# WhatAShot/Electrocardio-Panorama

Hardware: AMD Instinct MI355X
Metric: ECG-samples/sec (train step) (higher is better)
Workload: dtype f32 (conv products: fp32 operands split into fp16 hi+lo = 22-23 bits, block-scaled, 3 fp16 matrix products each, fp32 accumulate; fp32-class, not IEEE fp32)

## Files before the change

electrocardio_panorama_amd/csrc/conv_h2w.hip:

```cpp
#include <hip/hip_runtime.h>
#include <stdint.h>
#include <stdlib.h>

#include <type_traits>

#include "nefnet_hip.h"
#include "nef_common.h"


typedef float f32x16 __attribute__((ext_vector_type(16)));
typedef float f32x2 __attribute__((ext_vector_type(2)));
typedef _Float16 h16x8 __attribute__((ext_vector_type(8)));
typedef _Float16 h16x2 __attribute__((ext_vector_type(2)));
typedef unsigned u32x4 __attribute__((ext_vector_type(4)));
typedef unsigned u32x2 __attribute__((ext_vector_type(2)));

namespace {

constexpr int TT = 64;
constexpr int GP = TT * 2 + 8;
constexpr int XW = TT + 8;
constexpr int XP = XW * 2 + 8;
constexpr int X_PLANE = 64 * XP;
constexpr int gy_plane(int MCO) { return 64 * MCO * GP; }
constexpr int buf_bytes(int MCO) { return 2 * gy_plane(MCO) + 2 * X_PLANE; }

struct H2WArgs {
    const float* x;
    const float* gy;
    const float* in_scale;
    const float* pro_a;
    const float* pro_b;
    float* ws;
    const float* x_amax;
    const float* gy_amax;
    float* x_amax_next;
    float* gy_amax_next;
    int* clamped;
    int64_t x_bs, x_gs, gy_bs, gy_gs, sc_bs, sc_gs;
    int64_t x_end, gy_end;
    int B, T, G, Cig, Cog, pro_Bp, S, tps, n_tiles, m_tiles, c_tiles, teams;
    float x_scale, gy_scale;
    int xclamp;
};


__device__ __forceinline__ void split_pair_s(float x0, float x1, float s, unsigned& h, unsigned& l) {
    asm("v_fma_mixlo_f16 %0, %1, %2, 0 op_sel:[0,0,0] op_sel_hi:[0,0,0]" : "=v"(h) : "v"(x0), "v"(s));
    asm("v_fma_mixhi_f16 %0, %1, %2, 0 op_sel:[0,0,0] op_sel_hi:[0,0,0]" : "+v"(h) : "v"(x1), "v"(s));
    asm("v_fma_mixlo_f16 %0, %1, %2, -%3 op_sel:[0,0,0] op_sel_hi:[0,0,1]" : "=v"(l) : "v"(x0), "v"(s), "v"(h));
    asm("v_fma_mixhi_f16 %0, %1, %2, -%3 op_sel:[0,0,1] op_sel_hi:[0,0,1]" : "+v"(l) : "v"(x1), "v"(s), "v"(h));
}
__device__ __forceinline__ void split_one_s(float x0, float s, unsigned& h, unsigned& l) {
    asm("v_fma_mixlo_f16 %0, %1, %2, 0 op_sel:[0,0,0] op_sel_hi:[0,0,0]" : "=v"(h) : "v"(x0), "v"(s));
    asm("v_fma_mixlo_f16 %0, %1, %2, -%3 op_sel:[0,0,0] op_sel_hi:[0,0,1]" : "=v"(l) : "v"(x0), "v"(s), "v"(h));
}

__device__ __forceinline__ float scale_for(float m) {
    int e;
    (void)frexpf(m, &e);
    return ldexpf(1.f, 9 - e);
}

__device__ __forceinline__ float scale_from(const float* amax, float fallback) {
    float s = fallback != 0.f ? fallback : 1.f;
    if (amax) {
        const float m = amax[0];
        if (m > 0.f && m < 3e38f) {
            int e;
            (void)frexpf(m, &e);
            s = ldexpf(1.f, 9 - e);
        }
    }
    return s;
}

template <int K, int K0, int K1, int MCO, int KA>
__device__ __forceinline__ void h2w_chunk(const unsigned char* ga, const unsigned char* xa, int c, f32x16 (&acc)[MCO][KA]) {
    constexpr int PAD = (K - 1) / 2;
    constexpr int GY_PLANE = gy_plane(MCO);
    h16x8 fah[MCO], fal[MCO];
#pragma unroll
    for (int i = 0; i < MCO; ++i) {
        unsigned ah[4], al[4];
#pragma unroll
        for (int j = 0; j < 2; ++j) {
            const u32x2 vh = *reinterpret_cast<const u32x2*>(ga + i * 32 * GP + c * 32 + 8 * j);
            const u32x2 vl = *reinterpret_cast<const u32x2*>(ga + i * 32 * GP + GY_PLANE + c * 32 + 8 * j);
            ah[2 * j] = vh[0], ah[2 * j + 1] = vh[1];
            al[2 * j] = vl[0], al[2 * j + 1] = vl[1];
        }
        fah[i] = __builtin_bit_cast(h16x8, u32x4{ah[0], ah[1], ah[2], ah[3]});
        fal[i] = __builtin_bit_cast(h16x8, u32x4{al[0], al[1], al[2], al[3]});
    }
    unsigned wh[8], wl[8];
#pragma unroll
    for (int j = 0; j < 4; ++j) {
        const u32x2 vh = *reinterpret_cast<const u32x2*>(xa + c * 32 + 8 * j);
        const u32x2 vl = *reinterpret_cast<const u32x2*>(xa + X_PLANE + c * 32 + 8 * j);
        wh[2 * j] = vh[0], wh[2 * j + 1] = vh[1];
        wl[2 * j] = vl[0], wl[2 * j + 1] = vl[1];
    }
    __builtin_amdgcn_s_setprio(1);
#pragma unroll
    for (int k = K0; k < K1; ++k) {
        const int e0 = 4 + k - PAD;
        unsigned bh[4], bl[4];
#pragma unroll
        for (int j = 0; j < 4; ++j) {
            if ((e0 & 1) == 0) {
                bh[j] = wh[e0 / 2 + j];
                bl[j] = wl[e0 / 2 + j];
            } else {
                bh[j] = __builtin_amdgcn_alignbit(wh[(e0 + 1) / 2 + j], wh[(e0 - 1) / 2 + j], 16);
                bl[j] = __builtin_amdgcn_alignbit(wl[(e0 + 1) / 2 + j], wl[(e0 - 1) / 2 + j], 16);
            }
        }
        const h16x8 fbh = __builtin_bit_cast(h16x8, u32x4{bh[0], bh[1], bh[2], bh[3]});
        const h16x8 fbl = __builtin_bit_cast(h16x8, u32x4{bl[0], bl[1], bl[2], bl[3]});
#pragma unroll
        for (int i = 0; i < MCO; ++i) acc[i][k - K0] = __builtin_amdgcn_mfma_f32_32x32x16_f16(fah[i], fbh, acc[i][k - K0], 0, 0, 0);
#pragma unroll
        for (int i = 0; i < MCO; ++i) acc[i][k - K0] = __builtin_amdgcn_mfma_f32_32x32x16_f16(fah[i], fbl, acc[i][k - K0], 0, 0, 0);
#pragma unroll
        for (int i = 0; i < MCO; ++i) acc[i][k - K0] = __builtin_amdgcn_mfma_f32_32x32x16_f16(fal[i], fbh, acc[i][k - K0], 0, 0, 0);
    }
}

template <int K, int PRO, int MCO, int SPLIT>
__global__ __launch_bounds__(SPLIT ? 512 : 256, SPLIT ? 1 : 2) void conv_h2w_kernel(H2WArgs a) {
    constexpr bool UP = (PRO & 2) != 0, AFF = (PRO & 1) != 0;
    constexpr int NT = SPLIT ? 512 : 256;
    constexpr int ROWS_G = 64 * MCO;
    constexpr int GY_PLANE = gy_plane(MCO), BUF = buf_bytes(MCO);
    constexpr int KA = SPLIT == 1 ? (K + 1) / 2 : K;
    constexpr int NGQ = ROWS_G * (TT / 2) / NT;
    constexpr int NXQ = (64 * (XW / 2) + NT - 1) / NT;
    static_assert(SPLIT == 0 || MCO == 2, "the 512-thread forms are the 128-channel tile");
    extern __shared__ __attribute__((aligned(16))) unsigned char smem_w[];

    const int members = a.m_tiles * a.c_tiles;
    const int xcd = blockIdx.x & 7, q_ = blockIdx.x >> 3;
    const int member = q_ % members;
    const int team = (q_ / members) * 8 + xcd;
    if (team >= a.teams) return;
    const int g = team / a.S, sp = team % a.S;
    const int mt = member / a.c_tiles, ct = member % a.c_tiles;
    const int T = a.T, Tin = UP ? (T >> 1) : T;
    const int lane = threadIdx.x & 63, wave = threadIdx.x >> 6;
    const int lo = lane & 31, hi = lane >> 5;
    const int wave_u = __builtin_amdgcn_readfirstlane(wave);
    const int wt = wave_u >> 2;
    const int wm = (wave_u >> 1) & 1, wn = wave_u & 1;

    const int64_t per = ((int64_t)a.n_tiles + a.S - 1) / a.S;
    const int n_lo = (int)(per * sp);
    int n_hi = (int)(per * (sp + 1));
    if (n_hi > a.n_tiles) n_hi = a.n_tiles;

    float* const Wl = reinterpret_cast<float*>(smem_w);
    float rx_ = 0.f, rg_ = 0.f;
    auto share_pass = [&](const float sx, const float sg, const bool last) __attribute__((always_inline)) -> bool {
    float amax_x = 0.f, amax_g = 0.f;

    f32x16 acc[MCO][KA];
#pragma unroll
    for (int i = 0; i < MCO; ++i)
#pragma unroll
        for (int k = 0; k < KA; ++k)
#pragma unroll
            for (int r = 0; r < 16; ++r) acc[i][k][r] = 0.f;

    f32x2 gq[NGQ];
    f32x2 xq[NXQ][UP ? 2 : 1];
#define NEF_W_ISSUE(N)                                                                                               \
    {                                                                                                               \
        const int b_ = (N) / a.tps, t0_ = ((N) % a.tps) * TT;                                                       \
        const bool on_ = (N) < n_hi;                                                                                \
        const __amdgpu_buffer_rsrc_t grs = nef_rsrc_n(a.gy + (int64_t)b_ * a.gy_bs + (int64_t)g * a.gy_gs + (int64_t)(mt * ROWS_G) * T, \
                                                      on_ ? 0x7FFFFFFCu : 0u);                                      \
        _Pragma("unroll") for (int q = 0; q < NGQ; ++q) {                                                           \
            const int p = (int)threadIdx.x + NT * q;                                                                \
            const int row = p >> 5, t = t0_ + 2 * (p & 31);                                                         \
            gq[q] = nef_buf_f32x2(grs, t < T ? (unsigned)((row * T + t) * 4) : NEF_OOB, 0);                         \
        }                                                                                                           \
        const __amdgpu_buffer_rsrc_t xrs = nef_rsrc_n(a.x + (int64_t)b_ * a.x_bs + (int64_t)g * a.x_gs + (int64_t)(ct * 64) * Tin, \
                                                      on_ ? 0x7FFFFFFCu : 0u);                                      \
        _Pragma("unroll") for (int q = 0; q < NXQ; ++q) {                                                           \
            const int p = (int)threadIdx.x + NT * q;                                                                \
            const int row = p / (XW / 2), t = t0_ - 4 + 2 * (p % (XW / 2));                                         \
            const bool ok = p < 64 * (XW / 2) && t >= 0 && t < T;                                                   \
            if constexpr (UP) {                                                                                     \
                 \
                const int h_ = t >> 1;                                                                              \
                const int im = h_ > 0 ? h_ - 1 : 0, ip = h_ + 1 < Tin ? h_ + 1 : Tin - 1;                           \
                const float v0 = nef_buf_f32(xrs, ok ? (unsigned)((row * Tin + im) * 4) : NEF_OOB, 0);              \
                const float v1 = nef_buf_f32(xrs, ok ? (unsigned)((row * Tin + h_) * 4) : NEF_OOB, 0);              \
                const float v2 = nef_buf_f32(xrs, ok ? (unsigned)((row * Tin + ip) * 4) : NEF_OOB, 0);              \
                xq[q][0] = f32x2{v0, v1};                                                                           \
                xq[q][UP ? 1 : 0] = f32x2{v1, v2};                                                                  \
            } else {                                                                                                \
                xq[q][0] = nef_buf_f32x2(xrs, ok ? (unsigned)((row * T + t) * 4) : NEF_OOB, 0);                     \
            }                                                                                                       \
        }                                                                                                           \
    }
#define NEF_W_STORE(N, BUFP)                                                                                         \
    {                                                                                                               \
        const int b_ = (N) / a.tps, t0_ = ((N) % a.tps) * TT;                                                       \
        _Pragma("unroll") for (int q = 0; q < NGQ; ++q) {                                                           \
            const int p = (int)threadIdx.x + NT * q;                                                                \
            const int row = p >> 5, c2 = p & 31;                                                                    \
            amax_g = fmaxf(amax_g, fmaxf(fabsf(gq[q][0]), fabsf(gq[q][1])));                                        \
            unsigned h_, l_;                                                                                        \
            split_pair_s(gq[q][0], gq[q][1], sg, h_, l_);                                                           \
            unsigned char* p_ = (BUFP) + row * GP + c2 * 4;                                                         \
            *reinterpret_cast<unsigned*>(p_) = h_;                                                                  \
            *reinterpret_cast<unsigned*>(p_ + GY_PLANE) = l_;                                                       \
        }                                                                                                           \
        _Pragma("unroll") for (int q = 0; q < NXQ; ++q) {                                                           \
            const int p = (int)threadIdx.x + NT * q;                                                                \
            const int row = p / (XW / 2), c2 = p % (XW / 2), t = t0_ - 4 + 2 * c2;                                  \
            if (p < 64 * (XW / 2)) {                                                                                \
                const int ch = g * a.Cig + ct * 64 + row;                                                           \
                float v0, v1;                                                                                       \
                if constexpr (UP) {                                                                                 \
                    float s0 = xq[q][0][0], s1 = xq[q][0][1], s2 = xq[q][UP ? 1 : 0][1];                            \
                    if constexpr (AFF) {                                                                            \
                        const int pr = (b_ / a.pro_Bp) * a.G * a.Cig + ch;                                          \
                        const float pa = a.pro_a[pr], pb = a.pro_b[pr];                                             \
                        s0 = fmaxf(fmaf(s0, pa, pb), 0.f), s1 = fmaxf(fmaf(s1, pa, pb), 0.f), s2 = fmaxf(fmaf(s2, pa, pb), 0.f); \
                    }                                                                                               \
                     \
                    v0 = t > 0 ? (1.f - 0.75f) * s0 + 0.75f * s1 : s1;                                              \
                    v1 = (1.f - 0.25f) * s1 + 0.25f * s2;                                                           \
                } else {                                                                                            \
                    v0 = xq[q][0][0], v1 = xq[q][0][1];                                                             \
                    if constexpr (AFF) {                                                                            \
                        const int pr = (b_ / a.pro_Bp) * a.G * a.Cig + ch;                                          \
                        const float pa = a.pro_a[pr], pb = a.pro_b[pr];                                             \
                        v0 = fmaxf(fmaf(v0, pa, pb), 0.f), v1 = fmaxf(fmaf(v1, pa, pb), 0.f);                       \
                    }                                                                                               \
                }                                                                                                   \
                if (a.in_scale) {                                                                                   \
                    const float sc = a.in_scale[(int64_t)b_ * a.sc_bs + (int64_t)g * a.sc_gs + ct * 64 + row];      \
                    v0 *= sc, v1 *= sc;                                                                             \
                }                                                                                                   \
                if (t < 0 || t >= T) v0 = v1 = 0.f;                      \
                amax_x = fmaxf(amax_x, fmaxf(fabsf(v0), fabsf(v1)));                                                \
                unsigned h_, l_;                                                                                    \
                split_pair_s(v0, v1, sx, h_, l_);                                                                   \
                unsigned char* p_ = (BUFP) + 2 * GY_PLANE + row * XP + c2 * 4;                                      \
                *reinterpret_cast<unsigned*>(p_) = h_;                                                              \
                *reinterpret_cast<unsigned*>(p_ + X_PLANE) = l_;                                                    \
            }                                                                                                       \
        }                                                                                                           \
    }

    if (n_lo < n_hi) {
        NEF_W_ISSUE(n_lo)
        NEF_W_STORE(n_lo, smem_w)
    }
    __syncthreads();
    for (int n = n_lo; n < n_hi; ++n) {
        const unsigned char* const bufp = smem_w + ((n - n_lo) & 1) * BUF;
        NEF_W_ISSUE(n + 1)
        const unsigned char* const ga = bufp + (wm * MCO * 32 + lo) * GP + hi * 16;
        const unsigned char* const xa = bufp + 2 * GY_PLANE + (wn * 32 + lo) * XP + hi * 16;
        if constexpr (SPLIT == 1) {
            if (wt == 0) {
#pragma unroll 1
                for (int c = 0; c < TT / 16; ++c) h2w_chunk<K, 0, KA, MCO, KA>(ga, xa, c, acc);
            } else {
#pragma unroll 1
                for (int c = 0; c < TT / 16; ++c) h2w_chunk<K, KA, K, MCO, KA>(ga, xa, c, acc);
            }
        } else if constexpr (SPLIT == 2) {
#pragma unroll
            for (int cc = 0; cc < TT / 32; ++cc) h2w_chunk<K, 0, K, MCO, KA>(ga, xa, 2 * cc + wt, acc);
        } else {
#pragma unroll
            for (int c = 0; c < TT / 16; ++c) h2w_chunk<K, 0, K, MCO, KA>(ga, xa, c, acc);
        }
        if (n + 1 < n_hi) NEF_W_STORE(n + 1, smem_w + ((n + 1 - n_lo) & 1) * BUF)
        __syncthreads();
    }
#undef NEF_W_ISSUE
#undef NEF_W_STORE

#pragma unroll
    for (int o = 32; o > 0; o >>= 1) {
        amax_x = fmaxf(amax_x, __shfl_xor(amax_x, o, 64));
        amax_g = fmaxf(amax_g, __shfl_xor(amax_g, o, 64));
    }
    if (lane == 0) Wl[wave_u] = amax_x, Wl[8 + wave_u] = amax_g;
    __syncthreads();
    {
        float wx = 0.f, wg_ = 0.f;
#pragma unroll
        for (int i = 0; i < NT / 64; ++i) wx = fmaxf(wx, Wl[i]), wg_ = fmaxf(wg_, Wl[8 + i]);
        __syncthreads();
        if (!last && !(wx * sx < 65000.f && wg_ * sg < 65000.f) && wx < 3e38f && wg_ < 3e38f) {
            rx_ = wx, rg_ = wg_;
            return false;
        }
    }
    if (a.clamped && lane == 0 && !(amax_x * sx < 65000.f && amax_g * sg < 65000.f)) atomicAdd(a.clamped, 1);
    if (a.x_amax_next && lane == 0) {
        unsigned* const px = reinterpret_cast<unsigned*>(a.x_amax_next);
        unsigned* const pg = reinterpret_cast<unsigned*>(a.gy_amax_next);
        const unsigned bx = __builtin_bit_cast(unsigned, amax_x), bg = __builtin_bit_cast(unsigned, amax_g);
        if (amax_x < 3e38f && bx > __atomic_load_n(px, __ATOMIC_RELAXED)) atomicMax(px, bx);
        if (amax_g < 3e38f && bg > __atomic_load_n(pg, __ATOMIC_RELAXED)) atomicMax(pg, bg);
    }

    const float ds = 1.f / (sx * sg);
    const int ci = ct * 64 + wn * 32 + lo;
    const int spw = SPLIT == 2 ? 2 * sp + wt : sp;
    const int k0 = SPLIT == 1 ? wt * KA : 0;
    float* const wsp = a.ws + ((int64_t)spw * a.G + g) * K * a.Cog * a.Cig;
#pragma unroll
    for (int i = 0; i < MCO; ++i) {
        const int co0 = mt * ROWS_G + (wm * MCO + i) * 32 + 4 * hi;
#pragma unroll
        for (int k = 0; k < KA; ++k) {
            if (k0 + k < K) {
#pragma unroll
                for (int r = 0; r < 16; ++r)
                    wsp[((int64_t)(k0 + k) * a.Cog + co0 + (r & 3) + 8 * (r >> 2)) * a.Cig + ci] = acc[i][k][r] * ds;
            }
        }
    }
    return true;
    };
    const float sx0 = scale_from(a.x_amax, a.x_scale), sg0 = scale_from(a.gy_amax, a.gy_scale);
    if (!share_pass(sx0, sg0, false))
        (void)share_pass(rx_ * sx0 < 65000.f ? sx0 : scale_for(rx_), rg_ * sg0 < 65000.f ? sg0 : scale_for(rg_), true);
}

template <int K, int PRO, int MCO, int SPLIT>
int launch_h2w(const H2WArgs& a, hipStream_t st) {
    constexpr size_t lds = 2 * buf_bytes(MCO);
    static unsigned long long lds_set = 0;
    if (int e = nef_ensure_dyn_lds(reinterpret_cast<const void*>(&conv_h2w_kernel<K, PRO, MCO, SPLIT>), lds, &lds_set)) return e;
    const int members = a.m_tiles * a.c_tiles;
    const int teams8 = (a.teams + 7) / 8 * 8;
    const int64_t blocks = (int64_t)teams8 * members;
    if (blocks <= 0 || blocks > 0x7fffffff) return NEF_E_SHAPE;
    hipLaunchKernelGGL((conv_h2w_kernel<K, PRO, MCO, SPLIT>), dim3((unsigned)blocks), dim3(SPLIT ? 512 : 256), lds, st, a);
    return nef_launch_status();
}

struct H2WForm { int mco, split; };
H2WForm h2w_form(int Cog, int K) {
    (void)Cog, (void)K;
    return {1, 0};
}


constexpr int H2W2_64_MODES = 12;
typedef u32x4 u32x4_a4 __attribute__((aligned(4)));
typedef float f32x4 __attribute__((ext_vector_type(4)));

__device__ __forceinline__ unsigned extent_from(int64_t end_bytes, int64_t off_elems, bool on) {
    int64_t r = end_bytes - off_elems * 4;
    if (r < 0) r = 0;
    if (r > 0x7FFFFFFC) r = 0x7FFFFFFC;
    return on ? (unsigned)r : 0u;
}

template <int K, int WR, int GP, int XP, int G_PLANE, int X_PLANE>
__device__ __forceinline__ void h2w2_chunk(const unsigned char* ga, const unsigned char* xa, int c, f32x16 (&acc)[WR][K]) {
    constexpr int PAD = (K - 1) / 2;
    h16x8 fah[WR], fal[WR];
#pragma unroll
    for (int i = 0; i < WR; ++i) {
        fah[i] = __builtin_bit_cast(h16x8, *reinterpret_cast<const u32x4*>(ga + i * 32 * GP + c * 32));
        fal[i] = __builtin_bit_cast(h16x8, *reinterpret_cast<const u32x4*>(ga + i * 32 * GP + G_PLANE + c * 32));
    }
    unsigned wn_h[8], wn_l[8], wo_h[8], wo_l[8];
    constexpr bool NAT = K >= 1, ODD = K >= 3;
#pragma unroll
    for (int j = 0; j < 2; ++j) {
        if (NAT) {
            const u32x4 vh = *reinterpret_cast<const u32x4*>(xa + c * 32 + 16 * j);
            const u32x4 vl = *reinterpret_cast<const u32x4*>(xa + X_PLANE + c * 32 + 16 * j);
#pragma unroll
            for (int i = 0; i < 4; ++i) wn_h[4 * j + i] = vh[i], wn_l[4 * j + i] = vl[i];
        }
        if (ODD) {
            const u32x4 vh = *reinterpret_cast<const u32x4*>(xa + 2 * X_PLANE + c * 32 + 16 * j);
            const u32x4 vl = *reinterpret_cast<const u32x4*>(xa + 3 * X_PLANE + c * 32 + 16 * j);
#pragma unroll
            for (int i = 0; i < 4; ++i) wo_h[4 * j + i] = vh[i], wo_l[4 * j + i] = vl[i];
        }
    }
    h16x8 fbh[K], fbl[K];
#pragma unroll
    for (int k = 0; k < K; ++k) {
        const int e0 = 4 + k - PAD;
        const int d = (e0 & 1) ? (e0 - 1) / 2 : e0 / 2;
        if (e0 & 1) {
// ... 284 lines not shown
    if (producer) {
        if (a.clamped && lane == 0 && !(amax_x * sx < 65000.f && amax_g * sg < 65000.f)) atomicAdd(a.clamped, 1);
        if (a.x_amax_next && lane == 0) {
            unsigned* const px = reinterpret_cast<unsigned*>(a.x_amax_next);
            unsigned* const pg = reinterpret_cast<unsigned*>(a.gy_amax_next);
            const unsigned bx = __builtin_bit_cast(unsigned, amax_x), bg = __builtin_bit_cast(unsigned, amax_g);
            if (amax_x < 3e38f && bx > __atomic_load_n(px, __ATOMIC_RELAXED)) atomicMax(px, bx);
            if (amax_g < 3e38f && bg > __atomic_load_n(pg, __ATOMIC_RELAXED)) atomicMax(pg, bg);
        }
        return true;
    }

    const float ds = 1.f / (sx * sg);
    const int ci = ct * RX + wn * 32 + lo;
    float* const wsp = a.ws + ((int64_t)sp * a.G + g) * K * a.Cog * a.Cig;
#pragma unroll
    for (int i = 0; i < WR; ++i) {
        const int co0 = mt * RG + (wm + i) * 32 + 4 * hi;
#pragma unroll
        for (int k = 0; k < K; ++k)
#pragma unroll
            for (int r = 0; r < 16; ++r) wsp[((int64_t)k * a.Cog + co0 + (r & 3) + 8 * (r >> 2)) * a.Cig + ci] = acc[i][k][r] * ds;
    }
    return true;
    };
    const float sx0 = scale_from(a.x_amax, a.x_scale), sg0 = scale_from(a.gy_amax, a.gy_scale);
    if (!share_pass(sx0, sg0, false))
        (void)share_pass(rx_ * sx0 < 65000.f ? sx0 : scale_for(rx_), rg_ * sg0 < 65000.f ? sg0 : scale_for(rg_), true);
}

template <int K, int PRO, int WM, int WN, int WR, int TTv, int NP, int DEPTH>
int launch_h2w2(const H2WArgs& a, hipStream_t st) {
    constexpr size_t lds = 2 * (2 * (32 * WM) * (TTv * 2 + 16) + 4 * (32 * WN) * ((TTv + 8) * 2));
    static unsigned long long lds_set = 0;
    if (int e = nef_ensure_dyn_lds(reinterpret_cast<const void*>(&conv_h2w2_kernel<K, PRO, WM, WN, WR, TTv, NP, DEPTH>), lds, &lds_set)) return e;
    const int members = a.m_tiles * a.c_tiles;
    const int teams8 = (a.teams + 7) / 8 * 8;
    const int64_t blocks = (int64_t)teams8 * members;
    if (blocks <= 0 || blocks > 0x7fffffff) return NEF_E_SHAPE;
    hipLaunchKernelGGL((conv_h2w2_kernel<K, PRO, WM, WN, WR, TTv, NP, DEPTH>), dim3((unsigned)blocks), dim3(64 * (WM / WR * WN + NP)), lds, st, a);
    return nef_launch_status();
}

int h2w2_form(int Cog, int pro_mode) {
    if (Cog % 128 == 0) return 1;
    return ((H2W2_64_MODES >> pro_mode) & 1) ? 2 : 0;
}

}

extern "C" {

__attribute__((visibility("hidden"))) bool nef_h2w_ok(int B, int T, int Cig, int Cog, int K, int pro_mode) {
    return (K == 1 || K == 3 || K == 7) && B > 0 && T >= TT && T % 2 == 0 && Cig % 64 == 0 && Cog % 64 == 0 && pro_mode >= 0 &&
           (pro_mode <= 3 || (pro_mode <= 5 && Cog % 128 == 0)) && (K == 3 || pro_mode == 0);
}

__attribute__((visibility("hidden"))) int nef_h2w_splits(int B, int T, int G, int Cig, int Cog, int K, int pro_mode, int* partials) {
    const int v2 = h2w2_form(Cog, pro_mode & 3);
    const H2WForm f = h2w_form(Cog, K);
    const int tps = (T + TT - 1) / TT;
    const int64_t n_tiles = (int64_t)B * tps;
    const int units = v2 ? G * (Cog / (v2 == 1 ? 128 : 64)) * (Cig / 64) : G * (Cog / (64 * f.mco)) * (Cig / 64);
    const int resident = v2 ? 1 : (f.split ? 1 : 2);
    const int slots = resident * nef_cu_count();
    int S = slots / units;
    if (S > n_tiles) S = (int)n_tiles;
    if (S < 1) S = 1;
    if (partials) *partials = S * (!v2 && f.split == 2 ? 2 : 1);
    return S;
}

__attribute__((visibility("hidden"))) int nef_h2w_launch(const nef_bww_args& b, int S, hipStream_t st) {
    const int B = b.B, T = b.T, G = b.G, Cig = b.Cin_g, Cog = b.Cout_g, K = b.K;
    int pro_mode = b.pro_mode;
    if (!nef_h2w_ok(B, T, Cig, Cog, K, pro_mode)) return NEF_E_SHAPE;
    if ((b.x_amax_next == nullptr) != (b.gy_amax_next == nullptr)) return NEF_E_NULL;
    const H2WForm f = h2w_form(Cog, K);
    H2WArgs a;
    a.x = b.x, a.gy = b.gy, a.in_scale = b.in_scale, a.pro_a = b.pro_a, a.pro_b = b.pro_b, a.ws = (float*)b.ws;
    a.x_amax = b.x_amax, a.gy_amax = b.gy_amax, a.x_amax_next = b.x_amax_next, a.gy_amax_next = b.gy_amax_next, a.clamped = b.clamped;
    a.x_bs = b.x_bs, a.x_gs = b.x_gs, a.gy_bs = b.gy_bs, a.gy_gs = b.gy_gs, a.sc_bs = b.sc_bs, a.sc_gs = b.sc_gs;
    a.B = B, a.T = T, a.G = G, a.Cig = Cig, a.Cog = Cog, a.pro_Bp = b.pro_Bp, a.S = S;
    a.tps = (T + TT - 1) / TT;
    a.n_tiles = B * a.tps;
    a.m_tiles = Cog / (64 * f.mco), a.c_tiles = Cig / 64;
    a.teams = G * S;
    a.x_scale = b.x_scale, a.gy_scale = b.gy_scale;
    a.xclamp = (pro_mode >> 2) & 1;
    pro_mode &= 3;
    const int Tin = (pro_mode & 2) ? T / 2 : T;
    a.x_end = ((int64_t)(B - 1) * b.x_bs + (int64_t)(G - 1) * b.x_gs + (int64_t)Cig * Tin) * 4;
    a.gy_end = ((int64_t)(B - 1) * b.gy_bs + (int64_t)(G - 1) * b.gy_gs + (int64_t)Cog * T) * 4;
    if (a.xclamp && !h2w2_form(Cog, pro_mode)) return NEF_E_UNSUPPORTED;
    if (const int v2 = h2w2_form(Cog, pro_mode)) {
        a.m_tiles = Cog / (v2 == 1 ? 128 : 64), a.c_tiles = Cig / 64;
#define NEF_H2W2(KK, PP)                                                                                             \
    (v2 == 1 ? launch_h2w2<KK, PP, 4, 2, (KK == 7 ? 1 : 2), 64, (KK == 7 ? 4 : 8), (KK == 7 ? 1 : 2)>(a, st)               \
             : launch_h2w2<KK, PP, 2, 2, 1, 64, 8, (KK == 7 ? 1 : 2)>(a, st))
        if (K == 7) return NEF_H2W2(7, 0);
        if (K == 1) return NEF_H2W2(1, 0);
        switch (pro_mode) {
            case 0: return NEF_H2W2(3, 0);
            case 1: return NEF_H2W2(3, 1);
            case 2: return NEF_H2W2(3, 2);
            default: return NEF_H2W2(3, 3);
        }
#undef NEF_H2W2
    }
    if (K == 7) return launch_h2w<7, 0, 1, 0>(a, st);
    if (K == 1) return launch_h2w<1, 0, 1, 0>(a, st);
    return pro_mode == 0 ? launch_h2w<3, 0, 1, 0>(a, st) : launch_h2w<3, 1, 1, 0>(a, st);
}

}
```

electrocardio_panorama_amd/engine.py:

```python
import os

import torch
from . import _env

from . import ops
from .ops import GV

N_SEG, ROI_BINS = 7, 16
DROP_P = 0.2
BN_EPS, BN_MOM = 1e-5, 0.1


DROPOUT_SITES = ("W_encoder.layer1.0", "W_encoder.layer1.1", "W_encoder.layer1.2", "w_conv.0", "z1_conv.0",
                 "z2_conv1.0", "z2_conv2.0", "z2_conv2.2")


class DropCfg:

    def __init__(self, training, p=DROP_P, masks=None, seed=0, seed_dev=None):
        self.seed_dev = seed_dev
        self.on = bool(training) and p > 0.0
        self.p = p if self.on else 0.0
        self.scale = 1.0 / (1.0 - p) if self.on else 1.0
        self.masks = masks
# ... 545 lines not shown


def gen_ecg(P, Bf, z1, z2b, query_thetas, rois, chunk=8, half=False):
    V = z1.shape[1] // 128
    ops.BATCH_HINT = z1.shape[0]
    ops.amax_roll()
    z2r = ops.roi_unpool_fwd(z2b.contiguous(), rois, z1.shape[2])
    latent = ops.lead_mean(z1, z2r, V)
    if half:
        return sweep_eval_h(P, Bf, latent, query_thetas)
    return sweep(P, Bf, latent, query_thetas, False, chunk)


def _head_bwd(P, sv, g_outs, grads, side, relu_z1=False):
    B, V = sv["hB"], sv["hV"]
    like = sv["dec"][2]
    g_out = ops.stacked3(g_outs) if all(g is not None for g in g_outs) else None
    if g_out is None:
        parts = [g if g is not None else torch.zeros_like(like[0:B]) for g in g_outs]
        g_out = torch.cat([p_.contiguous() for p_ in parts], dim=0)
    gD, up, shared = decoder_bwd(sv["dec"], g_out, P, grads, side)
    gz2r = gz2b = None
    z2r, T = sv["z2r"], sv["latent"].shape[2]
    fused = z2r is None and gD.shape[2] == T and T <= ops.UNPOOL_MIX_MAX_T
    gz1_sum = None
    if z2r is None and not fused:
        z2r = ops.roi_unpool_fwd(sv["z2b"], sv["rois"], T)
    if fused:
        gz1, gz2b, gq, *rest = ops.mix_bwd_shared_unpool(gD, sv["latent"], sv["z1"], sv["z2b"], sv["rois"], sv["q"], V, sv["choice"],
                                                         relu_z1=relu_z1, chan_sum=relu_z1)
        gz1_sum = rest[0] if rest else None
    elif shared:
        gz1, gz2r, gq = ops.mix_bwd_shared_up(gD, sv["latent"], sv["z1"], z2r, sv["q"], V, sv["choice"],
                                              relu_z1=relu_z1)
    else:
        gz1, gz2r, gq = ops.mix_bwd(gD, sv["latent"], sv["z1"], z2r, sv["q"], V, sv["choice"], upsampled=up,
                                    relu_z1=relu_z1)
    gW2, gb2 = side.run(lambda: ops.theta_mlp_bwd(sv["q_theta"], gq, 256), gq)
    grads["mlp2.weight"], grads["mlp2.bias"] = gW2, gb2
    return gz1, gz2r, gz2b, gz1_sum


EARLY_HOOK = None


def _latents_bwd(P, sv, gz1, gz2r, grads, side, z1_pre_gated=False, early=False, gz2b=None, gz1_sum=None):
    B, V, T = sv["B"], sv["V"], sv["T"]
    ops.pack_many(_latent_pack_requests(P, V, T, sv["z2_win"], True))
    if gz2b is None:
        gz2b = ops.roi_unpool_bwd(gz2r, sv["rois"])
    gh3 = gz2b.view(B, 128 * V * N_SEG, 2 * ROI_BINS)
    gh2 = block_bwd(sv["blk_c22"], gh3, P, grads, side=side)
    gh2q = ops.convt2_deinterleave(gh2)
    gwt, gbt = side.run(lambda: ops.convt2_bwd_weight(sv["h1"], gh2, N_SEG * V, gyq=gh2q), sv["h1"], gh2, gh2q)
    grads["z2_conv2.1.weight"], grads["z2_conv2.1.bias"] = gwt, gbt
    gh1 = ops.convt2_bwd_data(gh2, P["z2_conv2.1.weight"], N_SEG * V, gyq=gh2q)
    gh0 = block_bwd(sv["blk_c20"], gh1, P, grads, side=side)
    genc = torch.empty(B, 128 * V, T, device=gz1.device, dtype=torch.float32)
    block_bwd(sv["blk_z1"], gz1, P, grads, out=GV.half(genc, V, 0), side=side, pre_gated=z1_pre_gated, gate_input=True,
              g2_chan_sum=gz1_sum if z1_pre_gated else None)
    win = sv["z2_win"]
    if win is not None:
        gz2c = ops.roi_align_bwd(gh0.view(B, 128 * V, N_SEG, ROI_BINS), sv["rois"], T, win[1], win[0])
        gxw = block_bwd(sv["blk_z2c"], gz2c, P, grads, side=side, gate_input=True)
        ops.window_scatter(gxw, GV.half(genc, V, 1), win[0])
    else:
        gz2c = ops.roi_align_bwd(gh0.view(B, 128 * V, N_SEG, ROI_BINS), sv["rois"], T)
        block_bwd(sv["blk_z2c"], gz2c, P, grads, out=GV.half(genc, V, 1), side=side, gate_input=True)
    gew = block_bwd(sv["blk_w_conv"], genc, P, grads, side=side, pre_gated=True, scale_bwd=True)
    if isinstance(gew, tuple):
        g, ge = gew
    else:
        g, ge = ops.chscale_bwd(gew, sv["w"], sv["e"], relu_x=True)
    gW1, gb1 = side.run(lambda: ops.theta_mlp_bwd(sv["in_theta"], ge, 128), ge)
    grads["mlp1.weight"], grads["mlp1.bias"] = gW1, gb1
    if early:
        if EARLY_HOOK is not None:
            EARLY_HOOK(P, grads, side)
        else:
            from . import parallel
            parallel.early_reduce(P, grads, getattr(side, "stream", None))
    for i in (2, 1, 0):
        g = block_bwd(sv["blk_enc"][i], g, P, grads, side=side, pre_gated=True, gate_input=(i > 0))
    grads["W_encoder.conv1.weight"] = ops.stem_bwd_weight(sv["x"], P["W_encoder.conv1.weight"], g)


def backward(P, sv, g_outs):
    grads = {}
    side = _side(sv["z1"].device, sv["z1"].numel())
    gz1, gz2r, gz2b, gz1_sum = _head_bwd(P, sv, g_outs, grads, side, relu_z1=True)
    _latents_bwd(P, sv, gz1, gz2r, grads, side, z1_pre_gated=True, early=True, gz2b=gz2b, gz1_sum=gz1_sum)
    side.join()
    return grads


def backward2(P, sv, g_outs):
    grads = {}
    side = _side(sv["z1"].device, sv["z1"].numel())
    gZ1, gZ2, _, _ = _head_bwd(P, sv, g_outs, grads, side)
    B, V = sv["fold"]
    T = gZ1.shape[2]
    gz1f = torch.empty(V * B, 128, T, device=gZ1.device, dtype=torch.float32)
    gz2rf = torch.empty_like(gz1f)
    for name, gZ, xin, gout in (("single_conv_z1.0", gZ1, sv["z1f"], gz1f), ("single_conv_z2.0", gZ2, sv["z2rf"], gz2rf)):
        wf = ops.pack_weight(P[name + ".weight"], 1, flip=True, T=T)
        gw = None
        for i in range(V):
# ... 13 lines not shown
```

electrocardio_panorama_amd/ops.py:

```python
import ctypes as C
import contextlib
import itertools
import os
from typing import NamedTuple, Optional

import torch
from . import _env

from . import _lib

N_SEG, ROI_BINS = 7, 16


def _p(t):
    return None if t is None else t.data_ptr()


def _stream():
    return torch.cuda.current_stream().cuda_stream


def _chk(t, dtype=torch.float32):
    assert t.is_cuda and t.dtype == dtype and t.is_contiguous(), (t.device, t.dtype, t.is_contiguous())
    return t
# ... 647 lines not shown

def poly_bwd_ok(G, Cog, Cig, T):
    Th = T // 2
    return (H2 and T % 2 == 0 and Th >= 128 and Cig % 64 == 0 and (2 * Cog) % 16 == 0 and h2_ok(3, 2 * Cog, Cig, Th) and
            _h2_fills(G, Cig, Th, 256, 128 if Cig % 128 == 0 else 64))


def conv_bwd_data_poly(gyv, w, Cig, bnb=None, site=None, phase_major=False):
    L = _lib.load()
    if phase_major:
        G, Cog, T = gyv.G, gyv.Cg // 2, 2 * gyv.T
    else:
        G, Cog, T = gyv.G, gyv.Cg, gyv.T
    Th = T // 2
    assert w.shape == (G * Cog, Cig, 3) and gyv.gs == Cog * T, "conv_bwd_data_poly: dense gradient rows"
    wp = pack_weight(w, G, flip=True, T=Th, site=w.data_ptr() if site is None else site, src=("poly", 0))
    if int(getattr(wp, "nef_wino", 0)) != 3:
        raise _lib.NefLibraryError("conv_bwd_data_poly: shape outside the split-fp16 kernel (ask poly_bwd_ok first)")
    xv = GV(gyv.t, gyv.B, G, 2 * Cog, Th, gyv.bs, gyv.gs, gyv.off)
    if bnb is not None and len(bnb) == 6:
        slots = conv_stats_buffer(wp, gyv.B, G, Cig, Th, gyv.t.device)
        bnb = None if slots is None else (*bnb, slots)
    g = conv(xv, wp, Cig, 3, role="conv_bwd_data", bnb=bnb, pro=None if phase_major else (4, None, None, 1),
             tag_extra="pm" if phase_major else "")
    g.nef_slots = bnb[6] if bnb is not None else None
    ba = [None] * 5 + [1, None, 0]
    if bnb is not None:
        ba = [_p(t) for t in bnb[:5]] + [bnb[5], _p(bnb[6][0]), bnb[6][1]]
    _lib.check(L.nef_poly_bwd_edge(gyv.ptr, _p(w), _p(g), gyv.B, G, Cog, Cig, T, *ba, int(phase_major), _stream()), "nef_poly_bwd_edge")
    return g


def poly_w_ok(B, G, Cog, Cig, T):
    Th = T // 2
    return (T % 4 == 0 and Cog % 64 == 0 and h2w_ok(3, Cig, 2 * Cog, Th, 1) and
            (BATCH_HINT is None or B * ((Th + 63) // 64) >= 8 * _H2_MIN_WGS))


def conv_bwd_weight_poly(xv, gy_pm, Cog, pro, xedge, site=None):
    L = _lib.load()
    G, Cig = xv.G, xv.Cg
    aff = pro is not None and bool(pro[0] & 1)
    gyv = GV.dense(gy_pm, G)
    gw2 = conv_bwd_weight(xv, gyv, 3, pro=(4 | int(aff), pro[1] if aff else None, pro[2] if aff else None, pro[3] if aff else 1),
                          site=site, h2=True, xedge=xedge)
    gw = torch.empty(G * Cog, Cig, 3, device=gy_pm.device, dtype=torch.float32)
    n = L.nef_poly_wgrad_fold_ws_bytes(xv.B, G, Cog, Cig)
    ws = torch.empty(n // 4, device=gy_pm.device, dtype=torch.float32)
    _lib.check(L.nef_poly_wgrad_fold(_p(gw2), _p(gy_pm), _p(xedge), _p(gw), _p(ws), n, xv.B, G, Cog, Cig, 2 * xv.T, _stream()),
               "nef_poly_wgrad_fold")
    return gw


def h2w_ok(K, Cig, Cog, T, pro_mode=0, in_scale=False):
    return (H2 and T % 2 == 0 and T >= 64 and Cig % 64 == 0 and Cog % 64 == 0 and
            (K == 3 or not pro_mode) and not (pro_mode and in_scale))


def conv_bwd_weight(xv, gyv, K, in_scale=None, pro=None, wino=None, site=None, h2=None, x_scale=0.0, gy_scale=0.0, xedge=None):
    L = _lib.load()
    B, T, G, Cig, Cog = xv.B, gyv.T, xv.G, xv.Cg, gyv.Cg
    dev = xv.t.device
    gw = torch.empty(G * Cog, Cig, K, device=dev, dtype=torch.float32)
    pm0 = pro[0] if pro is not None else 0
    a = _lib.BwwArgs()
    _operand(a, xv, in_scale, pro)
    a.gy, a.gy_bs, a.gy_gs, a.gw = gyv.ptr, gyv.bs, gyv.gs, _p(gw)
    a.B, a.T, a.G, a.Cin_g, a.Cout_g, a.K = B, T, G, Cig, Cog, K
    a.x_scale, a.gy_scale = float(x_scale), float(gy_scale)
    routed = False
    if h2 is None:
        h2 = (wino is None and h2w_ok(K, Cig, Cog, T, pm0, in_scale is not None) and
              (BATCH_HINT is None or B * ((T + 63) // 64) >= 8 * _H2_MIN_WGS))
    if h2:
        _bww_form(L, a, 3, dev, f"conv_bwd_weight (split-fp16): unsupported shape Cig={Cig} Cog={Cog} K={K} T={T}")
        if not (x_scale and gy_scale):
            st = _amax_state(dev)
            key = None
            if AMAX_SCOPE is not None and site is not None:
                occ = st["occ"]
                base = (AMAX_SCOPE, (site, "w"), "conv_bwd_weight", B, T)
                k = occ[base] = occ.get(base, 0) + 1
                key = base + (k,)
            i = _amax_index(st, key if key is not None else (None, "bww"), 2)
            nxt = st["nxt"].data_ptr() + 4 * i
            a.x_amax_next, a.gy_amax_next = nxt, nxt + 4
            if i not in st["ready"] or key is None:
                if torch.cuda.is_current_stream_capturing():
                    raise RuntimeError("split-fp16 weight gradient: a call site's first launch cannot be captured")
                st["nxt"][i:i + 2] = 0.0
                _bww(L, a)
                st["cur"][i:i + 2] = st["nxt"][i:i + 2]
                if key is not None:
                    flag = _note_tail(st, i, [(xv, in_scale, pro), (gyv, None, None)])
                    if _tail_mode() == "fp32" and int(flag.item()):
                        st["fp32"].add(i)
                        st["fallback"] += 1
                st["ready"].add(i)
            routed = i in st["fp32"]
            if not routed:
                st["used"] = True
                cur = st["cur"].data_ptr() + 4 * i
                a.x_amax, a.gy_amax, a.clamped = cur, cur + 4, st["clamped"].data_ptr()
        if not routed:
            tag = ("conv_bwd_weight", K, G, Cig, Cog, B, T) + (("up",) if pm0 & 2 else (("pw",) if pm0 & 4 else ()))
            ev = _timed(tag)
            if ev is not None:
                EXEC_FRAC[tag] = 0.0
                EXEC_FP16[tag] = 3.0
            _bww(L, a)
            _done(ev)
            return gw
    extra = ("up" if pm0 & 2 else "") + (("pw" if pm0 & 4 else "") + "f32" if routed else "")
    if routed:
        wino = False
    clamp = bool(pm0 & 4)
    if clamp:
        if xedge is None:
            raise _lib.NefLibraryError("conv_bwd_weight: pro_mode bit 2 on the fp32 kernels needs `xedge`")
        pm0 = a.pro_mode = pm0 & 3
    if wino is None:
        wino = (WINOGRAD and ((K == 3 and WINO_BW4) or (K == 7 and WINO_BW7)) and T % 2 == 0 and T >= 64
                and not (K == 7 and pm0))
    wino = 4 if wino else False
    assert wino or not pm0 or in_scale is None
    _bww_form(L, a, wino or 0, dev, f"conv_bwd_weight: unsupported shape Cig={Cig} Cog={Cog} K={K}")
# ... 68 lines not shown
    Cig, Cog = Ct // G, gy.shape[1] // G
    gw = torch.empty(G * Cig, Cog, 2, device=x.device, dtype=torch.float32)
    gb = torch.empty(G * Cog, device=x.device, dtype=torch.float32)
    n = L.nef_convt2_bwd_weight_ws_bytes(G, Cig, Cog)
    ws = workspace(n, x.device)
    _lib.check(L.nef_convt2_bwd_weight(_p(x), _p(gy), _p(gw), _p(gb), _p(ws), n, B, G, Cig, Cog, T, _stream()),
               "nef_convt2_bwd_weight")
    return gw, gb


def group_transpose(t, G, R, Cn):
    L = _lib.load()
    _chk(t)
    out = torch.empty_like(t)
    _lib.check(L.nef_group_transpose(_p(t), _p(out), G, R, Cn, _stream()), "nef_group_transpose")
    return out


def convt2_as_conv_weight(w, G):
    Cig, Cog = w.shape[0] // G, w.shape[1]
    return group_transpose(w, G, Cig, 2 * Cog).view(G * 2 * Cog, Cig, 1)


def convt2_deinterleave(gy):
    L = _lib.load()
    _chk(gy)
    B, Ct, To = gy.shape
    gyq = torch.empty(B, 2 * Ct, To // 2, device=gy.device, dtype=torch.float32)
    _lib.check(L.nef_convt2_deinterleave(_p(gy), _p(gyq), B, Ct, To // 2, _stream()), "nef_convt2_deinterleave")
    return gyq


def convt2_fwd(x, w, bias, G, fma=False):
    if fma:
        return _convt2_fma_fwd(x, w, bias, G)
    L = _lib.load()
    _chk(x), _chk(w), _chk(bias)
    B, Ct, T = x.shape
    Cog = w.shape[1]
    yq = conv(GV.dense(x, G), pack_weight(convt2_as_conv_weight(w, G), G), 2 * Cog, 1)
    y = torch.empty(B, G * Cog, 2 * T, device=x.device, dtype=torch.float32)
    _lib.check(L.nef_convt2_interleave(_p(yq), _p(bias), _p(y), B, G * Cog, T, _stream()), "nef_convt2_interleave")
    return y


def convt2_bwd_data(gy, w, G, fma=False, gyq=None):
    if fma:
        return _convt2_fma_bwd_data(gy, w, G)
    Cig = w.shape[0] // G
    gyq = convt2_deinterleave(gy) if gyq is None else gyq
    return conv(GV.dense(gyq, G), pack_weight(convt2_as_conv_weight(w, G), G, flip=True), Cig, 1, role="conv_bwd_data")


def convt2_bwd_weight(x, gy, G, fma=False, gyq=None):
    if fma:
        return _convt2_fma_bwd_weight(x, gy, G)
    B, Ct, T = x.shape
    Cig, Cog = Ct // G, gy.shape[1] // G
    gyq = convt2_deinterleave(gy) if gyq is None else gyq
    gwc = conv_bwd_weight(GV.dense(x, G), GV.dense(gyq, G), 1)
    gw = group_transpose(gwc.contiguous(), G, 2 * Cog, Cig).view(G * Cig, Cog, 2)
    return gw, chan_sum(gy)


def theta_mlp_fwd(theta, W, bias):
    L = _lib.load()
    _chk(theta), _chk(W), _chk(bias)
    N, O = theta.numel() // 2, W.shape[0]
    y = torch.empty(*theta.shape[:-1], O, device=theta.device, dtype=torch.float32)
    _lib.check(L.nef_theta_mlp_fwd(_p(theta), _p(W), _p(bias), _p(y), N, O, _stream()), "nef_theta_mlp_fwd")
    return y


def theta_mlp_bwd(theta, gy, O):
    L = _lib.load()
    _chk(theta), _chk(gy)
    N = theta.numel() // 2
    gW = torch.empty(O, 12, device=theta.device, dtype=torch.float32)
    gb = torch.empty(O, device=theta.device, dtype=torch.float32)
    _lib.check(L.nef_theta_mlp_bwd(_p(theta), _p(gy), _p(gW), _p(gb), N, O, _stream()), "nef_theta_mlp_bwd")
    return gW, gb


def theta_encode(theta):
    L = _lib.load()
    _chk(theta)
    N = theta.numel() // 2
    enc = torch.empty(*theta.shape[:-1], 12, device=theta.device, dtype=torch.float32)
    _lib.check(L.nef_theta_encode(_p(theta), _p(enc), N, _stream()), "nef_theta_encode")
    return enc


def chscale_fwd(x, s, s_bs=None):
    L = _lib.load()
    _chk(x)
    B, Ct, T = x.shape
    y = torch.empty_like(x)
    ev = _hbm("chscale_fwd", x, y)
    _lib.check(L.nef_chscale_fwd(_p(x), _p(s), Ct if s_bs is None else s_bs, _p(y), B, Ct, T, _stream()), "nef_chscale_fwd")
    _done(ev)
    return y


def slots_to_rows(slots, B):
    sl, nslot = slots
    out = torch.empty(B, sl.shape[0], device=sl.device, dtype=torch.float32)
    _lib.check(_lib.load().nef_slots_to_rows(_p(sl), nslot, _p(out), B, sl.shape[0], _stream()), "nef_slots_to_rows")
    return out


def chscale_bwd(gy, x, s, s_bs=None, relu_x=False):
    L = _lib.load()
    _chk(gy), _chk(x)
# ... 806 lines not shown
```

Baseline: 8869.

## Pack several short-T batch rows into one 64-column tile for split-fp16 weight grads

```diff
diff --git a/electrocardio_panorama_amd/csrc/conv_h2w.hip b/electrocardio_panorama_amd/csrc/conv_h2w.hip
--- a/electrocardio_panorama_amd/csrc/conv_h2w.hip
+++ b/electrocardio_panorama_amd/csrc/conv_h2w.hip
@@ -75,8 +75,8 @@
     return s;
 }
 
-template <int K, int K0, int K1, int MCO, int KA>
-__device__ __forceinline__ void h2w_chunk(const unsigned char* ga, const unsigned char* xa, int c, f32x16 (&acc)[MCO][KA]) {
+template <int K, int K0, int K1, int MCO, int KA, bool PACK = false>
+__device__ __forceinline__ void h2w_chunk(const unsigned char* ga, const unsigned char* xa, int c, f32x16 (&acc)[MCO][KA], unsigned pm = 0u) {
     constexpr int PAD = (K - 1) / 2;
     constexpr int GY_PLANE = gy_plane(MCO);
     h16x8 fah[MCO], fal[MCO];
@@ -116,6 +116,16 @@
                 bl[j] = __builtin_amdgcn_alignbit(wl[(e0 + 1) / 2 + j], wl[(e0 - 1) / 2 + j], 16);
             }
         }
+        if constexpr (PACK && K == 3) {
+            const unsigned f = pm >> (3 * c);
+            if (k == 0) {
+                const unsigned m0 = (f & 1u) ? 0xFFFF0000u : 0xFFFFFFFFu, m2 = (f & 2u) ? 0xFFFF0000u : 0xFFFFFFFFu;
+                bh[0] &= m0, bl[0] &= m0, bh[2] &= m2, bl[2] &= m2;
+            } else if (k == 2) {
+                const unsigned m1 = (f & 2u) ? 0x0000FFFFu : 0xFFFFFFFFu, m3 = (f & 4u) ? 0x0000FFFFu : 0xFFFFFFFFu;
+                bh[1] &= m1, bl[1] &= m1, bh[3] &= m3, bl[3] &= m3;
+            }
+        }
         const h16x8 fbh = __builtin_bit_cast(h16x8, u32x4{bh[0], bh[1], bh[2], bh[3]});
         const h16x8 fbl = __builtin_bit_cast(h16x8, u32x4{bl[0], bl[1], bl[2], bl[3]});
 #pragma unroll
@@ -127,9 +137,10 @@
     }
 }
 
-template <int K, int PRO, int MCO, int SPLIT>
+template <int K, int PRO, int MCO, int SPLIT, bool PACK = false>
 __global__ __launch_bounds__(SPLIT ? 512 : 256, SPLIT ? 1 : 2) void conv_h2w_kernel(H2WArgs a) {
     constexpr bool UP = (PRO & 2) != 0, AFF = (PRO & 1) != 0;
+    static_assert(!PACK || (PRO == 0 && SPLIT == 0 && (K == 1 || K == 3)), "packed short rows: plain K = 1 / 3 launches");
     constexpr int NT = SPLIT ? 512 : 256;
     constexpr int ROWS_G = 64 * MCO;
     constexpr int GY_PLANE = gy_plane(MCO), BUF = buf_bytes(MCO);
@@ -173,8 +184,42 @@
 
     f32x2 gq[NGQ];
     f32x2 xq[NXQ][UP ? 2 : 1];
+    int pk_gc = 0x7fffffff, pk_xc[PACK ? NXQ : 1];
+    unsigned pk_go = 0u, pk_xo[PACK ? NXQ : 1], pk_m = 0u;
+    if constexpr (PACK) {
+        const int cols = a.tps * T;
+        const int c = 2 * ((int)threadIdx.x & 31), j = c / T;
+        if (c < cols) pk_gc = c, pk_go = (unsigned)(((int64_t)j * a.gy_bs + (int64_t)((int)threadIdx.x >> 5) * T + (c - j * T)) * 4);
+#pragma unroll
+        for (int q = 0; q < NXQ; ++q) {
+            const int p = (int)threadIdx.x + NT * q;
+            const int row = p / (XW / 2), cc = 2 * (p % (XW / 2)) - 4;
+            const bool ok = p < 64 * (XW / 2) && cc >= 0 && cc < cols;
+            const int jj = ok ? cc / T : 0;
+            pk_xc[q] = ok ? cc : 0x7fffffff;
+            pk_xo[q] = ok ? (unsigned)(((int64_t)jj * a.x_bs + (int64_t)row * T + (cc - jj * T)) * 4) : NEF_OOB;
+        }
+#pragma unroll
+        for (int c16 = 0; c16 < TT / 16; ++c16) {
+            const int s0 = 16 * c16 + 8 * hi;
+            pk_m |= ((s0 % T == 0 ? 1u : 0u) | ((s0 + 4) % T == 0 ? 2u : 0u) | ((s0 + 8) % T == 0 ? 4u : 0u)) << (3 * c16);
+        }
+    }
 #define NEF_W_ISSUE(N)                                                                                               \
-    {                                                                                                               \
+    if constexpr (PACK) {                                                                                           \
+        const int b0_ = (N) * a.tps;                                                                                \
+        const bool on_ = (N) < n_hi;                                                                                \
+        const int nv_ = a.B - b0_ < a.tps ? a.B - b0_ : a.tps;                                                      \
+        const int lim_ = on_ ? nv_ * T : 0;               \
+        const __amdgpu_buffer_rsrc_t grs = nef_rsrc_n(a.gy + (int64_t)b0_ * a.gy_bs + (int64_t)g * a.gy_gs + (int64_t)(mt * ROWS_G) * T, \
+                                                      on_ ? 0x7FFFFFFCu : 0u);                                      \
+        _Pragma("unroll") for (int q = 0; q < NGQ; ++q)                                                             \
+            gq[q] = nef_buf_f32x2(grs, pk_gc < lim_ ? pk_go + (unsigned)(q * (NT / 32) * T * 4) : NEF_OOB, 0);      \
+        const __amdgpu_buffer_rsrc_t xrs = nef_rsrc_n(a.x + (int64_t)b0_ * a.x_bs + (int64_t)g * a.x_gs + (int64_t)(ct * 64) * T, \
+                                                      on_ ? 0x7FFFFFFCu : 0u);                                      \
+        _Pragma("unroll") for (int q = 0; q < NXQ; ++q)                                                             \
+            xq[q][0] = nef_buf_f32x2(xrs, pk_xc[q] < lim_ ? pk_xo[q] : NEF_OOB, 0);                                 \
+    } else {                                                                                                        \
         const int b_ = (N) / a.tps, t0_ = ((N) % a.tps) * TT;                                                       \
         const bool on_ = (N) < n_hi;                                                                                \
         const __amdgpu_buffer_rsrc_t grs = nef_rsrc_n(a.gy + (int64_t)b_ * a.gy_bs + (int64_t)g * a.gy_gs + (int64_t)(mt * ROWS_G) * T, \
@@ -245,7 +290,7 @@
                     const float sc = a.in_scale[(int64_t)b_ * a.sc_bs + (int64_t)g * a.sc_gs + ct * 64 + row];      \
                     v0 *= sc, v1 *= sc;                                                                             \
                 }                                                                                                   \
-                if (t < 0 || t >= T) v0 = v1 = 0.f;                      \
+                if (!PACK && (t < 0 || t >= T)) v0 = v1 = 0.f;       \
                 amax_x = fmaxf(amax_x, fmaxf(fabsf(v0), fabsf(v1)));                                                \
                 unsigned h_, l_;                                                                                    \
                 split_pair_s(v0, v1, sx, h_, l_);                                                                   \
@@ -279,7 +324,7 @@
             for (int cc = 0; cc < TT / 32; ++cc) h2w_chunk<K, 0, K, MCO, KA>(ga, xa, 2 * cc + wt, acc);
         } else {
 #pragma unroll
-            for (int c = 0; c < TT / 16; ++c) h2w_chunk<K, 0, K, MCO, KA>(ga, xa, c, acc);
+            for (int c = 0; c < TT / 16; ++c) h2w_chunk<K, 0, K, MCO, KA, PACK>(ga, xa, c, acc, pk_m);
         }
         if (n + 1 < n_hi) NEF_W_STORE(n + 1, smem_w + ((n + 1 - n_lo) & 1) * BUF)
         __syncthreads();
@@ -337,16 +382,16 @@
         (void)share_pass(rx_ * sx0 < 65000.f ? sx0 : scale_for(rx_), rg_ * sg0 < 65000.f ? sg0 : scale_for(rg_), true);
 }
 
-template <int K, int PRO, int MCO, int SPLIT>
+template <int K, int PRO, int MCO, int SPLIT, bool PACK = false>
 int launch_h2w(const H2WArgs& a, hipStream_t st) {
     constexpr size_t lds = 2 * buf_bytes(MCO);
     static unsigned long long lds_set = 0;
-    if (int e = nef_ensure_dyn_lds(reinterpret_cast<const void*>(&conv_h2w_kernel<K, PRO, MCO, SPLIT>), lds, &lds_set)) return e;
+    if (int e = nef_ensure_dyn_lds(reinterpret_cast<const void*>(&conv_h2w_kernel<K, PRO, MCO, SPLIT, PACK>), lds, &lds_set)) return e;
     const int members = a.m_tiles * a.c_tiles;
     const int teams8 = (a.teams + 7) / 8 * 8;
     const int64_t blocks = (int64_t)teams8 * members;
     if (blocks <= 0 || blocks > 0x7fffffff) return NEF_E_SHAPE;
-    hipLaunchKernelGGL((conv_h2w_kernel<K, PRO, MCO, SPLIT>), dim3((unsigned)blocks), dim3(SPLIT ? 512 : 256), lds, st, a);
+    hipLaunchKernelGGL((conv_h2w_kernel<K, PRO, MCO, SPLIT, PACK>), dim3((unsigned)blocks), dim3(SPLIT ? 512 : 256), lds, st, a);
     return nef_launch_status();
 }
 
@@ -737,15 +782,17 @@
 extern "C" {
 
 __attribute__((visibility("hidden"))) bool nef_h2w_ok(int B, int T, int Cig, int Cog, int K, int pro_mode) {
-    return (K == 1 || K == 3 || K == 7) && B > 0 && T >= TT && T % 2 == 0 && Cig % 64 == 0 && Cog % 64 == 0 && pro_mode >= 0 &&
+    const bool rows = T >= TT ? T % 2 == 0 : (T >= 8 && T % 4 == 0 && (K == 1 || K == 3) && pro_mode == 0);
+    return (K == 1 || K == 3 || K == 7) && B > 0 && rows && Cig % 64 == 0 && Cog % 64 == 0 && pro_mode >= 0 &&
            (pro_mode <= 3 || (pro_mode <= 5 && Cog % 128 == 0)) && (K == 3 || pro_mode == 0);
 }
 
 __attribute__((visibility("hidden"))) int nef_h2w_splits(int B, int T, int G, int Cig, int Cog, int K, int pro_mode, int* partials) {
-    const int v2 = h2w2_form(Cog, pro_mode & 3);
+    const bool pack = T < TT;
+    const int v2 = pack ? 0 : h2w2_form(Cog, pro_mode & 3);
     const H2WForm f = h2w_form(Cog, K);
     const int tps = (T + TT - 1) / TT;
-    const int64_t n_tiles = (int64_t)B * tps;
+    const int64_t n_tiles = pack ? nef_cdiv(B, TT / (T > 0 ? T : 1)) : (int64_t)B * tps;
     const int units = v2 ? G * (Cog / (v2 == 1 ? 128 : 64)) * (Cig / 64) : G * (Cog / (64 * f.mco)) * (Cig / 64);
     const int resident = v2 ? 1 : (f.split ? 1 : 2);
     const int slots = resident * nef_cu_count();
@@ -777,6 +824,15 @@
     const int Tin = (pro_mode & 2) ? T / 2 : T;
     a.x_end = ((int64_t)(B - 1) * b.x_bs + (int64_t)(G - 1) * b.x_gs + (int64_t)Cig * Tin) * 4;
     a.gy_end = ((int64_t)(B - 1) * b.gy_bs + (int64_t)(G - 1) * b.gy_gs + (int64_t)Cog * T) * 4;
+    if (T < TT) {
+        if (b.in_scale || pro_mode) return NEF_E_UNSUPPORTED;
+        a.tps = TT / T;
+        a.n_tiles = (B + a.tps - 1) / a.tps;
+        const int64_t lim = 0x7fffffff / 4;
+        if ((a.tps - 1) * b.x_bs + (int64_t)Cig * T >= lim || (a.tps - 1) * b.gy_bs + (int64_t)Cog * T >= lim || b.x_bs < 0 || b.gy_bs < 0)
+            return NEF_E_SHAPE;
+        return K == 1 ? launch_h2w<1, 0, 1, 0, true>(a, st) : launch_h2w<3, 0, 1, 0, true>(a, st);
+    }
     if (a.xclamp && !h2w2_form(Cog, pro_mode)) return NEF_E_UNSUPPORTED;
     if (const int v2 = h2w2_form(Cog, pro_mode)) {
         a.m_tiles = Cog / (v2 == 1 ? 128 : 64), a.c_tiles = Cig / 64;
diff --git a/electrocardio_panorama_amd/engine.py b/electrocardio_panorama_amd/engine.py
--- a/electrocardio_panorama_amd/engine.py
+++ b/electrocardio_panorama_amd/engine.py
@@ -621,7 +621,8 @@
     gh3 = gz2b.view(B, 128 * V * N_SEG, 2 * ROI_BINS)
     gh2 = block_bwd(sv["blk_c22"], gh3, P, grads, side=side)
     gh2q = ops.convt2_deinterleave(gh2)
-    gwt, gbt = side.run(lambda: ops.convt2_bwd_weight(sv["h1"], gh2, N_SEG * V, gyq=gh2q), sv["h1"], gh2, gh2q)
+    gwt, gbt = side.run(lambda: ops.convt2_bwd_weight(sv["h1"], gh2, N_SEG * V, gyq=gh2q, site=P["z2_conv2.1.weight"].data_ptr()),
+                        sv["h1"], gh2, gh2q)
     grads["z2_conv2.1.weight"], grads["z2_conv2.1.bias"] = gwt, gbt
     gh1 = ops.convt2_bwd_data(gh2, P["z2_conv2.1.weight"], N_SEG * V, gyq=gh2q)
     gh0 = block_bwd(sv["blk_c20"], gh1, P, grads, side=side)
diff --git a/electrocardio_panorama_amd/ops.py b/electrocardio_panorama_amd/ops.py
--- a/electrocardio_panorama_amd/ops.py
+++ b/electrocardio_panorama_amd/ops.py
@@ -723,9 +723,21 @@
     return gw
 
 
+def _h2w_packed(K, T, pro_mode=0, in_scale=False):
+    return K in (1, 3) and not pro_mode and not in_scale and 8 <= T < 64 and T % 4 == 0
+
+
 def h2w_ok(K, Cig, Cog, T, pro_mode=0, in_scale=False):
-    return (H2 and T % 2 == 0 and T >= 64 and Cig % 64 == 0 and Cog % 64 == 0 and
+    return (H2 and T % 2 == 0 and (T >= 64 or _h2w_packed(K, T, pro_mode, in_scale)) and Cig % 64 == 0 and Cog % 64 == 0 and
             (K == 3 or not pro_mode) and not (pro_mode and in_scale))
+
+
+def _h2w_fills(B, T, G, Cig, Cog):
+    if BATCH_HINT is None:
+        return True
+    if T < 64:
+        return -(-B // (64 // T)) * G * (Cog // 64) * (Cig // 64) >= 8 * _H2_MIN_WGS
+    return B * ((T + 63) // 64) >= 8 * _H2_MIN_WGS
 
 
 def conv_bwd_weight(xv, gyv, K, in_scale=None, pro=None, wino=None, site=None, h2=None, x_scale=0.0, gy_scale=0.0, xedge=None):
@@ -741,8 +753,7 @@
     a.x_scale, a.gy_scale = float(x_scale), float(gy_scale)
     routed = False
     if h2 is None:
-        h2 = (wino is None and h2w_ok(K, Cig, Cog, T, pm0, in_scale is not None) and
-              (BATCH_HINT is None or B * ((T + 63) // 64) >= 8 * _H2_MIN_WGS))
+        h2 = wino is None and h2w_ok(K, Cig, Cog, T, pm0, in_scale is not None) and _h2w_fills(B, T, G, Cig, Cog)
     if h2:
         _bww_form(L, a, 3, dev, f"conv_bwd_weight (split-fp16): unsupported shape Cig={Cig} Cog={Cog} K={K} T={T}")
         if not (x_scale and gy_scale):
@@ -917,13 +928,14 @@
     return conv(GV.dense(gyq, G), pack_weight(convt2_as_conv_weight(w, G), G, flip=True), Cig, 1, role="conv_bwd_data")
 
 
-def convt2_bwd_weight(x, gy, G, fma=False, gyq=None):
+def convt2_bwd_weight(x, gy, G, fma=False, gyq=None, site=None):
     if fma:
         return _convt2_fma_bwd_weight(x, gy, G)
     B, Ct, T = x.shape
     Cig, Cog = Ct // G, gy.shape[1] // G
     gyq = convt2_deinterleave(gy) if gyq is None else gyq
-    gwc = conv_bwd_weight(GV.dense(x, G), GV.dense(gyq, G), 1)
+    gwc = conv_bwd_weight(GV.dense(x, G), GV.dense(gyq, G), 1, site=site,
+                          h2=False if (site is None and T < 64) else None)
     gw = group_transpose(gwc.contiguous(), G, 2 * Cog, Cig).view(G * Cig, Cog, 2)
     return gw, chan_sum(gy)
 
```

New measurement: 8954, median of 6. Within noise of the previous version (+1.0%).
